# Danderson123/Amira

Measured on AMD Instinct MI355X. Metric: gene-mers/s to corrected GeneMerGraph, higher is better.
Workload: dtype int32; 1 GPU; synthetic 1M reads x 60 genes, k=5, 20k-gene vocab: build + error-correction sweep (build, filter(3,1), correct, build, clip(5), correct, build); reads_per_gpu=1000000, genes_per_read=60, k=5, vocab=20000, gene_mers_per_gpu=56000000, final_nodes=472478, final_edges=1054844, multi_gpu=n/a

## Files before the change

### amira_amd/csrc/amg_correct.h

```cpp
#pragma once
#include "amg_device.h"

enum { RC_SKIP = 0, RC_COPY = 1, RC_DROP = 2, RC_TRIM = 3, RC_GAPPED = 4, RC_KEEP_ORIG = 5 };

struct CorrArgs {
  const int* tokens;
  const long long* read_off;
  const int* tok_node;
  const signed char* tok_dir;
  const unsigned char* read_fix;
  const long long* p0s;
  const long long* p0e;
  const long long* p1s;
  const long long* p1e;
  long long n0;
  const long long* pos_off;
  const long long* read_len;
  long long n_reads;
  int k, flip, have_pos;
  unsigned int* gflag;
  unsigned long long* max_bound;
  unsigned long long* lmask;
  unsigned long long* n_runs;
  unsigned char* cls;
// ... 36 lines not shown

__device__ __forceinline__ unsigned long long gap_run_ends(unsigned long long lv, int start, int end) {
  const unsigned long long inside =
      (end >= 63 ? ~0ull : ((1ull << (end + 1)) - 1ull)) & ~((1ull << (start & 63)) - 1ull);
  return ~lv & inside & (lv >> 1);
}
__device__ __forceinline__ void gap_run_terminals(unsigned long long lv, int i, int& ps, int& pe) {
  ps = 63 - __clzll((long long)(lv & ((1ull << i) - 1ull)));
  pe = i + 1;
}

struct GapArgs {
  CorrArgs a;
  GView g;
  const GapRec* rec;
  const int* gapped_reads;
  long long n_gapped;
  int* pool;
  unsigned long long pool_cap;
  unsigned long long* pool_used;
  unsigned long long* status;
  int* cand;
  unsigned int cand_stride;
  unsigned char* final_cls;
  unsigned char* need_slow;
  const int* gq;
  const int4* qres;
  const int* qpool;
};

#define GF_MAXW 128
#define GF_MAXGAP 16
#define GF_POOL 384
#define GF_CAND 136
#define GF_MAXCOMBO 256
#define GM_INLINE 64
#define LEAN_CHUNK 32
#define CLS_READS 64
#define PACK_READS 64
enum {
  GS_NOT_TRIED = 1,
  GS_WINDOWS = 2,
  GS_RUNS = 3,
  GS_MEMO_UNFIT = 4,
  GS_RECORDS = 5,
  GS_COMBOS = 6,
  GS_CAND = 7,
  GS_CODES = 8
};
enum {
  GL_NO_SLOTS = 1,
  GL_ANSWERS = 2,
  GL_LONG = 3,
  GL_OTHER = 4,
  GL_CODES = 5
};

#define NWF_MAX_M 64
#define NWF_MAX_N 128
__device__ __forceinline__ bool nw_fast_ok(long long N, long long M) {
  return N <= NWF_MAX_N && M <= NWF_MAX_M && N > 0 && M > 0;
}

struct __attribute__((aligned(16))) NwRec {
  int r, M, N, pad;
  long long t0, dst;
  long long pdst;
  long long poff;
};

struct NwArgs {
  CorrArgs a;
  const NwRec* rec;
  long long* o_gs;
  long long* o_ge;
  const int* gapped_reads;
  long long n_gapped;
  const unsigned char* final_cls;
  const long long* big_off;
  unsigned char* big_buf;
  int allow_fast;
  int shortcuts;
  unsigned char* route;
};
enum { NW_ROUTE_NONE = 0, NW_ROUTE_EQUAL = 1, NW_ROUTE_CERT = 2, NW_ROUTE_FILL = 3, NW_ROUTE_LDS = 4, NW_ROUTE_GLOBAL = 5 };

struct PackArgs {
  CorrArgs a;
  const long long* new_idx;
  const long long* new_off;
  const unsigned char* final_cls;
  int* o_tok;
  long long* o_off;
  int* o_orig;
  unsigned char* o_changed;
  long long* o_src;
  const long long* pos_new;
  long long* o_posoff;
  long long* o_rl;
  long long out_reads, out_tokens;
  unsigned long long* dead_kept;
};

struct CorrSwitches {
  bool gap_memo;
  bool fast_gapped;
  bool lean_gapped;
  int fast_nw;
  int nw_shortcuts;
  const char* node_bound;
  bool routes;
  const char* gap_pool;
  const char* memo_spill;
};

struct CorrScratch {
  size_t per_read = 0;
  unsigned char *cls = nullptr, *final_cls = nullptr;
  int *r_start = nullptr, *r_end = nullptr;
  long long *nw_size = nullptr, *nw_off = nullptr;
  unsigned int *bound = nullptr, *new_len = nullptr, *flag = nullptr;
  long long *tmp_off = nullptr, *new_idx = nullptr, *new_off = nullptr;
  int* tmp_tok = nullptr;
  long long *plen = nullptr, *poffs = nullptr, *pos_new = nullptr;
  unsigned long long *max_bound = nullptr, *n_general = nullptr;
  unsigned long long* n_runs = nullptr;
  unsigned long long* dead_kept = nullptr;
  bool count_alive = false;
  DevBuf* glist = nullptr;
  DevBuf* cand = nullptr;
  DevBuf* pool = nullptr;
  DevBuf* need_slow = nullptr;
};

struct CorrCounts {
  long long tmp_total = 0, n_gapped = 0, total_runs = 0;
  unsigned long long max_bound = 0;
  bool carry = false;
  long long out_reads = 0, out_tokens = 0, big_total = 0, pos_total = 0;
  unsigned long long n_general = 0;
  long long n_queries = 0;
  int pool_retries = 0;
  bool lean_ran = false, fast_ran = false, memo = false;
};

static void fill_pos_args(amg_ctx* c, CorrArgs& a) {
  a.p0s = c->have_pos ? c->gene_start.as<long long>() : nullptr;
  a.p0e = c->have_pos ? c->gene_end.as<long long>() : nullptr;
  a.p1s = c->pos1_s.as<long long>();
  a.p1e = c->pos1_e.as<long long>();
  a.n0 = c->pos_n0;
  a.pos_off = (c->have_pos && !c->pos_identity) ? c->pos_off.as<long long>() : nullptr;
}

void corr_classify_launch(amg_ctx* c, const CorrArgs& a);
int corr_gapped(amg_ctx* c, const CorrSwitches& sw, const CorrScratch& S, const CorrArgs& a, CorrCounts& n);
int corr_nw_sizes(amg_ctx* c, const CorrSwitches& sw, const CorrScratch& S, const CorrArgs& a, long long n_gapped,
                  FetchList& shape);
int corr_grow_pos_pools(amg_ctx* c, const CorrCounts& n);
int corr_positions(amg_ctx* c, const CorrSwitches& sw, const CorrScratch& S, const CorrArgs& a, const CorrCounts& n,
                   unsigned char* route = nullptr);

int routes_begin(amg_ctx* c);
int routes_gapped(amg_ctx* c, const CorrScratch& S, const CorrCounts& n, const unsigned char* need_slow, const int* gq);
int routes_nw(amg_ctx* c, const CorrScratch& S, const CorrCounts& n);
int routes_end(amg_ctx* c, const CorrCounts& n);
```

### amira_amd/csrc/amg_correct.hip

```cpp
#include "amg_correct.h"

__global__ __launch_bounds__(256) void k_count_alive(const unsigned char* __restrict__ alive, long long n,
                                                     unsigned long long* out) {
  __shared__ unsigned int s_part[4];
  unsigned int c = 0;
  for (long long i = ((long long)blockIdx.x * blockDim.x + threadIdx.x) * 4; i < n; i += (long long)gridDim.x * blockDim.x * 4) {
    if (i + 4 <= n) {
      const unsigned int w = *reinterpret_cast<const unsigned int*>(alive + i);
      c += __popc(w & 0x01010101u);
    } else {
      for (long long j = i; j < n; ++j) c += alive[j] ? 1u : 0u;
    }
  }
  for (int d = 32; d > 0; d >>= 1) c += (unsigned int)__shfl_xor((int)c, d, 64);
  if ((threadIdx.x & 63) == 0) s_part[threadIdx.x >> 6] = c;
  __syncthreads();
  if (threadIdx.x == 0 && (s_part[0] | s_part[1] | s_part[2] | s_part[3]))
    atomicAdd(out, (unsigned long long)s_part[0] + s_part[1] + s_part[2] + s_part[3]);
}

__global__ __launch_bounds__(256) void k_corr_pack(PackArgs A) {
  const CorrArgs& a = A.a;
  const int lane = threadIdx.x & 63;
  const long long r = ((long long)blockIdx.x * 4 + (threadIdx.x >> 6)) * PACK_READS + lane;
  if (blockIdx.x == 0 && threadIdx.x == 0) A.o_off[A.out_reads] = A.out_tokens;
  long long dst = 0, src = 0;
  int n = 0;
  unsigned int dead = 0;
  if (r < a.n_reads && a.new_len[r] > 0) {
    dst = A.new_off[r];
    n = (int)a.new_len[r];
    const unsigned char fc = A.final_cls[r];
    if (fc == RC_KEEP_ORIG) {
      const long long nw = a.read_off[r + 1] - a.read_off[r] - a.k + 1;
      dead = nw <= 64 ? (unsigned int)(nw - __popcll(a.lmask[r])) : (unsigned int)nw;
    }
    long long poff = 0;
    if (fc == RC_GAPPED) {
      src = a.tmp_off[r] | (1ll << 62);
      if (a.have_pos) poff = A.pos_new[r];
    } else {
      const long long cut = fc == RC_TRIM ? a.r_start[r] : 0;
      src = a.read_off[r] + cut;
      if (a.have_pos) poff = (a.pos_off ? a.pos_off[r] : a.read_off[r]) + cut;
    }
    const long long q = A.new_idx[r];
    A.o_off[q] = dst;
    A.o_orig[q] = (int)r;
    A.o_changed[q] = (fc == RC_TRIM || fc == RC_GAPPED) ? 1 : 0;
    A.o_src[q] = fc == RC_GAPPED ? -1ll : src;
    if (a.have_pos) A.o_posoff[q] = poff;
    if (a.read_len) A.o_rl[q] = a.read_len[r];
  }
  if (__ballot(dead != 0u) != 0ull) {
    for (int d = 32; d > 0; d >>= 1) dead += (unsigned int)__shfl_xor((int)dead, d, 64);
    if (lane == 0) atomicAdd(A.dead_kept + 16 * (blockIdx.x & 15), (unsigned long long)dead);
  }
  if (__ballot(n > 0) == 0ull) return;
  for (int j0 = 0; j0 < PACK_READS; j0 += 4) {
    const int* sp[4];
    long long d[4];
    int nn[4], vt[4];
#pragma unroll
    for (int j = 0; j < 4; ++j) {
      nn[j] = __builtin_amdgcn_readlane(n, j0 + j);
      const long long sj = bcast_i64(src, j0 + j);
      d[j] = bcast_i64(dst, j0 + j);
      sp[j] = ((sj >> 62) & 1 ? a.tmp_tok : a.tokens) + (sj & ~(1ll << 62));
    }
#pragma unroll
    for (int j = 0; j < 4; ++j)
      if (lane < nn[j]) vt[j] = sp[j][lane];
#pragma unroll
    for (int j = 0; j < 4; ++j)
      if (lane < nn[j]) A.o_tok[d[j] + lane] = vt[j];
#pragma unroll
    for (int j = 0; j < 4; ++j)
      for (int i = 64 + lane; i < nn[j]; i += 64)
        A.o_tok[d[j] + i] = sp[j][i];
  }
}

static CorrSwitches read_switches() {
  auto is_one = [](const char* name) {
    const char* v = getenv(name);
    return v && v[0] == '1';
  };
  CorrSwitches sw;
  sw.gap_memo = !is_one("AMG_NO_GAP_MEMO");
  sw.fast_gapped = !is_one("AMG_NO_FAST_GAPPED");
  sw.lean_gapped = !is_one("AMG_NO_LEAN_GAPPED");
  sw.fast_nw = !is_one("AMG_NO_FAST_NW");
  sw.nw_shortcuts = !is_one("AMG_NW_NO_SHORTCUT");
  sw.node_bound = getenv("AMG_TEST_NODE_BOUND");
  sw.routes = is_one("AMG_CORR_ROUTES");
  sw.gap_pool = getenv("AMG_TEST_GAP_POOL");
  sw.memo_spill = getenv("AMG_TEST_MEMO_SPILL");
  return sw;
}

static int plan_per_read(amg_ctx* c, CorrScratch& S) {
  const size_t per_read = (size_t)(c->n_reads + 2);
  AMGCHK(c->s0.ensure(per_read * (1 + 1) + 64));
  AMGCHK(c->s1.ensure(per_read * sizeof(int) * 2 + per_read * sizeof(long long) * 2 + 64));
  AMGCHK(c->s2.ensure(per_read * sizeof(unsigned int) * 3));
  AMGCHK(c->s3.ensure(per_read * sizeof(long long) * 3));
  AMGCHK(c->gm_mask.ensure(per_read * sizeof(unsigned long long)));
  AMGCHK(c->gm_ctr.ensure((16 + 256 + 256 + 16) * sizeof(unsigned long long)));
  S.per_read = per_read;
  S.cls = c->s0.as<unsigned char>();
  S.final_cls = S.cls + per_read;
  S.r_start = c->s1.as<int>();
  S.r_end = S.r_start + per_read;
  S.nw_size = reinterpret_cast<long long*>(((uintptr_t)(S.r_end + per_read) + 15) & ~(uintptr_t)15);
  S.nw_off = S.nw_size + per_read;
  S.bound = c->s2.as<unsigned int>();
  S.new_len = S.bound + per_read;
  S.flag = S.new_len + per_read;
  S.tmp_off = c->s3.as<long long>();
  S.new_idx = S.tmp_off + per_read;
  S.new_off = S.new_idx + per_read;
  S.max_bound = S.n_general = c->status.as<unsigned long long>() + ST_MISC;
  S.n_runs = c->gm_ctr.as<unsigned long long>() + 16;
  S.dead_kept = S.n_runs + 256;
  S.count_alive = c->n_nodes >= (1ll << 20);
  S.glist = &c->c_orig;
  S.cand = &c->c_gstart;
  S.pool = &c->c_gend;
  S.need_slow = &c->c_changed;
  return AMG_OK;
}

static int plan_staging(amg_ctx* c, CorrScratch& S, long long tmp_total) {
  AMGCHK(c->c_tokens_buf.ensure((size_t)(tmp_total + 4) * sizeof(int)));
  AMGCHK(c->s4.ensure((size_t)(tmp_total + 4) * sizeof(int)));
  S.tmp_tok = c->s4.as<int>();
  return AMG_OK;
}

static int plan_positions(amg_ctx* c, CorrScratch& S, long long n_gapped) {
  AMGCHK(c->s5.ensure((size_t)(2 * (n_gapped + 2) + c->n_reads + 2) * sizeof(long long)));
  S.plen = c->s5.as<long long>();
  S.poffs = S.plen + (n_gapped + 2);
  S.pos_new = S.poffs + (n_gapped + 2);
  return AMG_OK;
}

static void corr_args(amg_ctx* c, const CorrScratch& S, CorrArgs& a) {
  a.tokens = c->tokens.as<int>();
  a.read_off = c->read_off.as<long long>();
  a.tok_node = c->tok_node.as<int>();
  a.tok_dir = c->tok_dir.as<signed char>();
  a.read_fix = c->read_fix.as<unsigned char>();
  fill_pos_args(c, a);
  a.read_len = c->have_read_len ? c->read_len.as<long long>() : nullptr;
  a.n_reads = c->n_reads;
  a.k = c->k;
  a.flip = c->two_v - 1;
  a.have_pos = c->have_pos ? 1 : 0;
  a.gflag = S.flag;
  a.max_bound = S.max_bound;
  a.lmask = c->gm_mask.as<unsigned long long>();
  a.n_runs = S.n_runs;
  a.cls = S.cls;
  a.cls_final = S.final_cls;
  a.r_start = S.r_start;
  a.r_end = S.r_end;
  a.bound = S.bound;
  a.tmp_off = S.tmp_off;
  a.new_len = S.new_len;
  a.tmp_tok = S.tmp_tok;
}

static int corr_classify(amg_ctx* c, const CorrScratch& S, const CorrArgs& a, CorrCounts& n) {
  hipStream_t st = c->stream;
  const long long R = c->n_reads;
// ... 156 lines not shown
```

### amira_amd/csrc/amg_correct_nw.hip

```cpp
#include "amg_correct.h"

#define NW_LDS_N 1024
#define NW_LDS_CELLS 16384
__global__ __launch_bounds__(64) void k_corr_nw(NwArgs A) {
  __shared__ unsigned char s_ptr[NW_LDS_CELLS];
  __shared__ int s_diag[3 * (NW_LDS_N + 1)];
  __shared__ unsigned char s_ops[2 * NW_LDS_N];
  const CorrArgs& a = A.a;
  const long long gi = blockIdx.x;
  if (gi >= A.n_gapped) return;
  const long long r = A.rec[gi].r;
  const long long pdst = A.rec[gi].pdst;
  if (A.final_cls[r] == RC_KEEP_ORIG) return;
  const int lane = threadIdx.x;
  const long long t0 = a.read_off[r];
  const int M = (int)(a.read_off[r + 1] - t0);
  const int N = (int)a.new_len[r];
  if (A.allow_fast && nw_fast_ok(N, M)) return;
  const long long dst = a.tmp_off[r];
  const int* x = a.tmp_tok + dst;
  const int* y = a.tokens + t0;
  const long long *ogs, *oge;
  pos_base(a, A.rec[gi].poff, ogs, oge);
  unsigned char* P = s_ptr;
  int* dg = s_diag;
  unsigned char* ops = s_ops;
  const bool small = (N <= NW_LDS_N && M <= NW_LDS_N && (long long)N * M <= NW_LDS_CELLS);
  if (!small) {
    unsigned char* base = A.big_buf + A.big_off[gi];
    P = base;
    ops = base + (long long)N * M;
    dg = reinterpret_cast<int*>(base + (((long long)N * M + N + M + 15) & ~15ll));
  }
  int* d0 = dg;
  int* d1 = d0 + (N + 1);
  int* d2 = d1 + (N + 1);
  for (int d = 0; d <= N + M - 2; ++d) {
    int ilo = d - (M - 1) > 0 ? d - (M - 1) : 0;
    int ihi = d < N - 1 ? d : N - 1;
    for (int i = ilo + lane; i <= ihi; i += 64) {
      int j = d - i;
      int f_dd = (i == 0 && j == 0) ? 0 : (i == 0 ? -(j - 1) : (j == 0 ? -(i - 1) : d0[i]));
      int f_im1 = (i == 0) ? -j : d1[i];
      int f_jm1 = (j == 0) ? -i : d1[i + 1];
      int s_diag_ = f_dd + (x[i] == y[j] ? 1 : 0);
      int s_left = f_im1 - 1;
      int s_up = f_jm1 - 1;
      int best = s_diag_;
      unsigned char ptr = 0;
      if (s_left >= best) { best = s_left; ptr = 1; }
      if (s_up >= best) { best = s_up; ptr = 2; }
      d2[i + 1] = best;
      P[(long long)i * M + j] = ptr;
    }
    __syncthreads();
    int* t = d0; d0 = d1; d1 = d2; d2 = t;
  }
  if (lane != 0) return;
  int n_ops = 0;
  int i = N - 1, j = M - 1;
  while (i >= 0 && j >= 0) {
    unsigned char p = P[(long long)i * M + j];
    ops[n_ops++] = p;
    if (p == 0) { --i; --j; }
    else if (p == 1) --i;
    else --j;
  }
  while (i >= 0) { ops[n_ops++] = 1; --i; }
  while (j >= 0) { ops[n_ops++] = 2; --j; }
  const long long NONE = (long long)0x8000000000000000ull;
  int xi = 0, yj = 0, cur = 0, out = 0;
  for (int o = n_ops - 1; o >= 0; --o) {
    unsigned char p = ops[o];
    if (p == 0) {
      if (x[xi] == y[yj]) {
        A.o_gs[pdst + out] = ogs[cur];
        A.o_ge[pdst + out] = oge[cur];
        ++cur;
      } else {
        A.o_gs[pdst + out] = NONE;
        A.o_ge[pdst + out] = NONE;
      }
      ++out; ++xi; ++yj;
    } else if (p == 1) {
      A.o_gs[pdst + out] = NONE;
      A.o_ge[pdst + out] = NONE;
      ++out; ++xi;
    } else {
      ++cur; ++yj;
    }
  }
  long long prev_end = 0;
  const long long rl = a.read_len ? a.read_len[r] : 0;
  for (int q = 0; q < N; ++q) {
    long long sv = A.o_gs[pdst + q], ev = A.o_ge[pdst + q];
    if (ev != NONE) prev_end = ev;
    if (sv == NONE && ev == NONE) {
      long long nxt = NONE;
      for (int w = q + 1; w < N; ++w)
        if (A.o_gs[pdst + w] != NONE) { nxt = A.o_gs[pdst + w]; break; }
      A.o_gs[pdst + q] = prev_end;
      A.o_ge[pdst + q] = (nxt != NONE) ? nxt : rl - 1;
    }
  }
}



#define NWF_WPB 1
struct NwfLds {
  int x[NWF_MAX_N];
  unsigned int opw[(NWF_MAX_N + NWF_MAX_M) / 16 + 1];
  long long gs[NWF_MAX_N];
  long long ge[NWF_MAX_N];
  long long ogs[NWF_MAX_M];
  long long oge[NWF_MAX_M];
};

__device__ __forceinline__ void nw_fast_read(const NwArgs& A, long long gi, int lane, NwfLds& S) {
  int (*s_x)[NWF_MAX_N] = &S.x;
  unsigned int (*s_opw)[(NWF_MAX_N + NWF_MAX_M) / 16 + 1] = &S.opw;
  long long (*s_gs)[NWF_MAX_N] = &S.gs;
  long long (*s_ge)[NWF_MAX_N] = &S.ge;
  long long (*s_ogs)[NWF_MAX_M] = &S.ogs;
  long long (*s_oge)[NWF_MAX_M] = &S.oge;
  const CorrArgs& a = A.a;
  const int wv = 0;
  const NwRec q = A.rec[gi];
  const int N = __builtin_amdgcn_readfirstlane(q.N);
  if (N == 0) return;
  const int M = __builtin_amdgcn_readfirstlane(q.M);
  const long long r = q.r, t0 = q.t0, dst = q.dst, pdst = q.pdst;
  int* X = s_x[wv];
  unsigned int* OPW = s_opw[wv];
  long long* GS = s_gs[wv];
  long long* GE = s_ge[wv];
  long long* OGS = s_ogs[wv];
  long long* OGE = s_oge[wv];
  const int x0 = lane < N ? a.tmp_tok[dst + lane] : -2;
  const int x1 = lane + 64 < N ? a.tmp_tok[dst + lane + 64] : -2;
  const int yj = lane < M ? a.tokens[t0 + lane] : -1;
  const long long *pgs, *pge;
  pos_base(a, q.poff, pgs, pge);
  const long long ogs = lane < M ? pgs[lane] : 0;
  const long long oge = lane < M ? pge[lane] : 0;
  const long long rl = a.read_len ? a.read_len[r] : 0;
  if (lane < N) X[lane] = x0;
  if (lane + 64 < N) X[lane + 64] = x1;
  OGS[lane] = ogs;
  OGE[lane] = oge;
  const long long NONE = (long long)0x8000000000000000ull;
  bool diagonal = false;
  int route = NW_ROUTE_FILL;
  if (N == M) {
    const unsigned long long mm = __ballot(lane < N && x0 != yj);
    const int m = __popcll(mm);
    diagonal = m <= 1;
    const int x_next = __shfl_down(x0, 1, 64), y_next = __shfl_down(yj, 1, 64);
    const unsigned long long eq_a = __ballot(lane < N - 1 && x0 == y_next);
    const unsigned long long eq_b = __ballot(lane < N - 1 && x_next == yj);
    if (m == 2) {
      const int b = 63 - __clzll((long long)mm);
      const unsigned long long upto_b = (1ull << b) - 1ull;
      diagonal = (eq_a & upto_b) != upto_b && (eq_b & upto_b) != upto_b;
    } else if (m == 3 || m == 4) {
      const unsigned long long dmask = ~mm & (N == 64 ? ~0ull : ((1ull << N) - 1ull));
      const unsigned long long below = (1ull << lane) - 1ull;
      const int prefD = __popcll(dmask & below);
      const int sufD = lane >= 63 ? 0 : __popcll(dmask >> (lane + 1));
      const int ID = (int)0x80000000 / 2;
      int best = ID;
#pragma unroll
      for (int side = 0; side < 2; ++side) {
        const int prefS = __popcll((side == 0 ? eq_a : eq_b) & below);
        int g = lane < N ? prefD - prefS + (lane == 0 ? 1 : 0) : ID;
        g = max(g, __builtin_amdgcn_update_dpp(ID, g, 0x111, 0xf, 0xf, false));
        g = max(g, __builtin_amdgcn_update_dpp(ID, g, 0x112, 0xf, 0xf, false));
        g = max(g, __builtin_amdgcn_update_dpp(ID, g, 0x114, 0xf, 0xf, false));
        g = max(g, __builtin_amdgcn_update_dpp(ID, g, 0x118, 0xf, 0xf, false));
        g = max(g, __builtin_amdgcn_update_dpp(ID, g, 0x142, 0xa, 0xf, false));
        g = max(g, __builtin_amdgcn_update_dpp(ID, g, 0x143, 0xc, 0xf, false));
        int h = lane < N ? g + prefS + sufD - 2 : ID;
        for (int d = 32; d > 0; d >>= 1) h = max(h, __shfl_xor(h, d, 64));
        best = max(best, h);
      }
      diagonal = best < N - m;
    }
    diagonal = diagonal && A.shortcuts != 0;
    if (diagonal) route = NW_ROUTE_EQUAL;
    if (diagonal && lane < N) {
      const bool match = ((mm >> lane) & 1ull) == 0ull;
      const int cur = __popcll(~mm & ((1ull << lane) - 1ull));
      GS[lane] = match ? OGS[cur] : NONE;
      GE[lane] = match ? OGE[cur] : NONE;
    }
  }
  if (!diagonal && A.shortcuts != 0 && N <= M && N >= 2) {
    int s_off = 0x7fffffff;
    bool ok = true;
    unsigned long long matched = 0ull;
    for (int i = 0; i < N && ok; ++i) {
      const int g = __builtin_amdgcn_readlane(x0, i);
      const unsigned long long at = __ballot(lane < M && yj == g);
      if (at != 0ull) {
        const int si = __ffsll((long long)at) - 1 - i;
        ok = (at & (at - 1ull)) == 0ull && (s_off == 0x7fffffff || si == s_off);
        s_off = si;
        matched |= 1ull << i;
      }
    }
    ok = ok && s_off != 0x7fffffff && s_off >= 0 && s_off <= M - N && __popcll(matched) >= 2;
    if (ok) {
      diagonal = true;
      route = NW_ROUTE_CERT;
      if (lane < N) {
// ... 37 lines not shown
    {
      int i = N - 1, j = M - 1;
      unsigned int pack = 0;
  #pragma unroll
      for (int blk = NWF_MAX_N / 16 - 1; blk >= 0; --blk) {
        while (i >= blk * 16 && j >= 0) {
          const unsigned int w = (unsigned int)__builtin_amdgcn_readlane((int)ptrs[blk], j);
          const unsigned int p = (w >> ((i & 15) * 2)) & 3u;
          pack |= p << ((n_ops & 15) * 2);
          if ((n_ops & 15) == 15) {
            if (lane == 0) OPW[n_ops >> 4] = pack;
            pack = 0;
          }
          ++n_ops;
          if (p == 0) { --i; --j; }
          else if (p == 1) --i;
          else --j;
        }
      }
      while (i >= 0) {
        pack |= 1u << ((n_ops & 15) * 2);
        if ((n_ops & 15) == 15) {
          if (lane == 0) OPW[n_ops >> 4] = pack;
          pack = 0;
        }
        ++n_ops;
        --i;
      }
      while (j >= 0) {
        pack |= 2u << ((n_ops & 15) * 2);
        if ((n_ops & 15) == 15) {
          if (lane == 0) OPW[n_ops >> 4] = pack;
          pack = 0;
        }
        ++n_ops;
        --j;
      }
      if ((n_ops & 15) != 0 && lane == 0) OPW[n_ops >> 4] = pack;
    }
    wave_sync();
    int base_x = 0, base_y = 0, base_cur = 0;
    for (int c0 = 0; c0 < n_ops; c0 += 64) {
      const int f = c0 + lane;
      const bool in = f < n_ops;
      const int g = in ? n_ops - 1 - f : 0;
      const unsigned int op = in ? (OPW[g >> 4] >> ((g & 15) * 2)) & 3u : 3u;
      const bool isx = in && (op == 0 || op == 1), isy = in && (op == 0 || op == 2);
      const unsigned long long lt = (1ull << lane) - 1ull;
      const unsigned long long bx = __ballot(isx), by = __ballot(isy);
      const int xi = base_x + __popcll(bx & lt), yy = base_y + __popcll(by & lt);
      const int ysel = __shfl(yj, yy < 64 ? yy : 0, 64);
      const bool match = in && op == 0 && X[xi < NWF_MAX_N ? xi : 0] == ysel;
      const bool inc = in && (op == 2 || match);
      const unsigned long long bc = __ballot(inc);
      const int cur = base_cur + __popcll(bc & lt);
      if (isx) {
        GS[xi] = match ? OGS[cur < NWF_MAX_M ? cur : 0] : NONE;
        GE[xi] = match ? OGE[cur < NWF_MAX_M ? cur : 0] : NONE;
      }
      base_x += __popcll(bx);
      base_y += __popcll(by);
      base_cur += __popcll(bc);
    }
  }
  wave_sync();
  if (A.route && lane == 0) A.route[gi] = (unsigned char)route;
  for (int q = lane; q < N; q += 64) {
    long long sv = GS[q], ev = GE[q];
    if (sv == NONE && ev == NONE) {
      long long prev_end = 0;
      for (int w = q - 1; w >= 0; --w)
        if (GE[w] != NONE) { prev_end = GE[w]; break; }
      long long nxt = NONE;
      for (int w = q + 1; w < N; ++w)
        if (GS[w] != NONE) { nxt = GS[w]; break; }
      sv = prev_end;
      ev = (nxt != NONE) ? nxt : rl - 1;
    }
    A.o_gs[pdst + q] = sv;
    A.o_ge[pdst + q] = ev;
  }
}

__global__ __launch_bounds__(64 * NWF_WPB) void k_corr_nw_fast(NwArgs A) {
  __shared__ NwfLds s_lds;
  if ((long long)blockIdx.x < A.n_gapped) nw_fast_read(A, (long long)blockIdx.x, (int)threadIdx.x, s_lds);
}

__global__ void k_nw_sizes(const int* __restrict__ gapped, long long n_gapped,
                           const long long* __restrict__ read_off, const unsigned int* __restrict__ new_len,
                           const long long* __restrict__ tmp_off, const long long* __restrict__ new_off,
                           const unsigned char* __restrict__ final_cls, long long* __restrict__ size,
                           int allow_fast, unsigned long long* n_general, NwRec* __restrict__ rec,
                           const long long* __restrict__ pos_off, long long* __restrict__ plen) {
  long long gi = (long long)blockIdx.x * blockDim.x + threadIdx.x;
  if (gi >= n_gapped) return;
  long long r = gapped[gi];
  long long N = new_len[r], M = read_off[r + 1] - read_off[r];
  {
    NwRec q;
    q.r = (int)r;
    q.M = (int)(M > 0x7fffffff ? 0x7fffffff : M);
    q.N = (final_cls[r] != RC_KEEP_ORIG && allow_fast && nw_fast_ok(N, M)) ? (int)N : 0;
    q.pad = 0;
    q.t0 = read_off[r];
    q.dst = tmp_off[r];
    q.pdst = 0;
    q.poff = pos_off ? pos_off[r] : read_off[r];
    rec[gi] = q;
    plen[gi] = final_cls[r] != RC_KEEP_ORIG ? N : 0;
  }
  bool small = (N <= NW_LDS_N && M <= NW_LDS_N && N * M <= NW_LDS_CELLS);
  long long bytes = 0;
  if (!small && final_cls[r] != RC_KEEP_ORIG)
    bytes = ((N * M + N + M + 15) & ~15ll) + ((3 * (N + 1) * 4 + 15) & ~15ll);
  size[gi] = bytes;
  if (final_cls[r] != RC_KEEP_ORIG && !(allow_fast && nw_fast_ok(N, M))) atomicAdd(n_general, 1ull);
}


__global__ void k_nw_place(long long n_gapped, const long long* __restrict__ poffs, long long base, long long n0,
                           NwRec* __restrict__ rec, long long* __restrict__ pos_new) {
  long long gi = (long long)blockIdx.x * blockDim.x + threadIdx.x;
  if (gi >= n_gapped) return;
  const long long at = base + poffs[gi];
  rec[gi].pdst = at;
  pos_new[rec[gi].r] = n0 + at;
}

static int grow_keep(amg_ctx* c, DevBuf& b, size_t need, size_t used) {
  if (need <= b.cap && !b.borrowed) return AMG_OK;
  DevBuf nb;
  AMGCHK(nb.ensure(need + need / 2));
  if (used && b.p) HIPCHK(hipMemcpyAsync(nb.p, b.p, used, hipMemcpyDeviceToDevice, c->stream));
  HIPCHK(hipStreamSynchronize(c->stream));
  b.release();
  b = nb;
  return AMG_OK;
}

int corr_nw_sizes(amg_ctx* c, const CorrSwitches& sw, const CorrScratch& S, const CorrArgs& a, long long n_gapped,
                  FetchList& shape) {
  {
    ClearList cl;
    cl.add(S.nw_size, (size_t)(n_gapped + 1) * sizeof(long long));
    cl.add(S.plen, (size_t)(n_gapped + 1) * sizeof(long long));
    cl.add(S.n_general, sizeof(unsigned long long));
    AMGCHK(clear_many(c, cl));
  }
  AMGCHK(c->nw_rec.ensure((size_t)(n_gapped + 1) * sizeof(NwRec)));
  hipLaunchKernelGGL(k_nw_sizes, dim3(nblk(n_gapped, 256)), dim3(256), 0, c->stream, S.glist->as<int>(),
                     n_gapped, a.read_off, S.new_len, S.tmp_off, S.new_off, S.final_cls, S.nw_size, sw.fast_nw,
                     S.n_general, c->nw_rec.as<NwRec>(), a.pos_off, S.plen);
  AMGCHK(prim_exscan_i64_pair(c, S.nw_size, S.nw_off, S.plen, S.poffs, (size_t)n_gapped));
  shape.add(S.nw_off + n_gapped);
  shape.add(S.poffs + n_gapped);
  shape.add(S.n_general);
  return AMG_OK;
}

int corr_grow_pos_pools(amg_ctx* c, const CorrCounts& n) {
  AMGCHK(c->nw_big.ensure((size_t)n.big_total + 64));
  const size_t used = (size_t)c->pos1_used * sizeof(long long);
  const size_t need = (size_t)(c->pos1_used + n.pos_total + 64) * sizeof(long long);
  AMGCHK(grow_keep(c, c->pos1_s, need, used));
  AMGCHK(grow_keep(c, c->pos1_e, need, used));
  return AMG_OK;
}

int corr_positions(amg_ctx* c, const CorrSwitches& sw, const CorrScratch& S, const CorrArgs& a, const CorrCounts& n,
                   unsigned char* route) {
  hipStream_t st = c->stream;
  const long long n_gapped = n.n_gapped;
  hipLaunchKernelGGL(k_nw_place, dim3(nblk(n_gapped, 256)), dim3(256), 0, st, n_gapped, S.poffs,
                     (long long)c->pos1_used, (long long)c->pos_n0, c->nw_rec.as<NwRec>(), S.pos_new);
  NwArgs W;
  W.a = a;
  W.rec = c->nw_rec.as<NwRec>();
  W.o_gs = c->pos1_s.as<long long>();
  W.o_ge = c->pos1_e.as<long long>();
  W.gapped_reads = nullptr;
  W.n_gapped = n_gapped;
  W.final_cls = S.final_cls;
  W.big_off = S.nw_off;
  W.big_buf = c->nw_big.as<unsigned char>();
  W.allow_fast = sw.fast_nw;
  W.shortcuts = sw.nw_shortcuts;
  W.route = route;
  if (W.allow_fast)
    hipLaunchKernelGGL(k_corr_nw_fast, dim3((unsigned int)n_gapped), dim3(64 * NWF_WPB), 0, st, W);
  if (n.n_general > 0)
    hipLaunchKernelGGL(k_corr_nw, dim3((unsigned int)n_gapped), dim3(64), 0, st, W);
  return AMG_OK;
}

struct NwProbeLoan {
  amg_ctx* c;
  DevBuf gene_start, gene_end, pos_off, pos1_s, pos1_e;
  bool have_pos, pos_identity;
  int64_t pos_n0, pos1_used;
  explicit NwProbeLoan(amg_ctx* ctx)
      : c(ctx), gene_start(ctx->gene_start), gene_end(ctx->gene_end), pos_off(ctx->pos_off), pos1_s(ctx->pos1_s),
        pos1_e(ctx->pos1_e), have_pos(ctx->have_pos), pos_identity(ctx->pos_identity), pos_n0(ctx->pos_n0),
        pos1_used(ctx->pos1_used) {
    c->gene_start = c->gene_end = c->pos_off = c->pos1_s = c->pos1_e = DevBuf();
  }
  ~NwProbeLoan() {
    c->gene_start.release(), c->gene_end.release(), c->pos_off.release(), c->pos1_s.release(), c->pos1_e.release();
    c->gene_start = gene_start, c->gene_end = gene_end, c->pos_off = pos_off, c->pos1_s = pos1_s, c->pos1_e = pos1_e;
    c->have_pos = have_pos, c->pos_identity = pos_identity, c->pos_n0 = pos_n0, c->pos1_used = pos1_used;
  }
};
struct NwProbeBufs {
  DevBuf tokens, read_off, tmp_tok, tmp_off, new_len, final_cls, read_len, glist, sizes, places, route;
  ~NwProbeBufs() {
    for (DevBuf* b : {&tokens, &read_off, &tmp_tok, &tmp_off, &new_len, &final_cls, &read_len, &glist, &sizes, &places,
                      &route})
      b->release();
  }
};
static int probe_up(DevBuf& b, const void* src, size_t bytes, size_t room = 0) {
  AMGCHK(b.ensure(bytes + room + 16));
  if (bytes) HIPCHK(hipMemcpy(b.p, src, bytes, hipMemcpyHostToDevice));
  return AMG_OK;
}

#define NWP_GUARD 64
#define NWP_GUARD_PRE 8
#define NWP_N0_POOLED 5
extern "C" int amg_nw_probe(amg_ctx* c, int64_t n_pairs, const int32_t* x_tok, const int64_t* x_off, const int32_t* y_tok,
                            const int64_t* y_off, const int64_t* y_start, const int64_t* y_end, const int64_t* read_len,
                            const uint8_t* keep_orig, int flags, int64_t* out_start, int64_t* out_end, uint8_t* route,
                            int64_t* state) {
  if (!c || n_pairs < 1 || n_pairs > (1ll << 20) || !x_off || !y_tok || !y_off || !y_start || !y_end || !route || !state ||
      flags < 0 || flags > 7 || x_off[0] != 0 || y_off[0] != 0)
    return amg_fail(AMG_E_ARG, "nw_probe: bad arguments");
  long long want_pos = 0, want_big = 0;
  for (int64_t p = 0; p < n_pairs; ++p) {
    const long long N = x_off[p + 1] - x_off[p], M = y_off[p + 1] - y_off[p];
    const bool keep = keep_orig && keep_orig[p];
    if (N < 0 || M < 1 || (N < 1 && !keep) || N > (1 << 24) || M > (1 << 24))
      return amg_fail(AMG_E_ARG, "nw_probe: pair %lld has %lld corrected and %lld original genes", (long long)p, N, M);
    if (keep) continue;
    want_pos += N;
    if (!(N <= NW_LDS_N && M <= NW_LDS_N && N * M <= NW_LDS_CELLS)) want_big += N * M + 16 * (N + M) + 64;
    if (want_big > (1ll << 30)) return amg_fail(AMG_E_ARG, "nw_probe: more than 1 GiB of matrix scratch");
  }
  const long long total_x = x_off[n_pairs], total_y = y_off[n_pairs];
  if (total_x > 0 && !x_tok) return amg_fail(AMG_E_ARG, "nw_probe: no corrected genes");
  if (want_pos > 0 && (!out_start || !out_end)) return amg_fail(AMG_E_ARG, "nw_probe: no room for the positions");
  for (long long i = 0; i < total_x; ++i)
    if (x_tok[i] < 0) return amg_fail(AMG_E_ARG, "nw_probe: negative corrected gene at %lld", i);
  for (long long i = 0; i < total_y; ++i)
    if (y_tok[i] < 0) return amg_fail(AMG_E_ARG, "nw_probe: negative original gene at %lld", i);
  HIPCHK(hipSetDevice(c->device));

  const bool pooled = (flags & 4) != 0;
  NwProbeLoan loan(c);
  NwProbeBufs B;
  CorrSwitches sw = {};
  sw.fast_nw = (flags & 1) ? 0 : 1;
  sw.nw_shortcuts = (flags & 2) ? 0 : 1;
  std::vector<unsigned int> new_len((size_t)n_pairs);
  std::vector<unsigned char> cls((size_t)n_pairs);
  std::vector<int> glist((size_t)n_pairs);
  for (int64_t p = 0; p < n_pairs; ++p) {
    new_len[p] = (unsigned int)(x_off[p + 1] - x_off[p]);
    cls[p] = (keep_orig && keep_orig[p]) ? RC_KEEP_ORIG : RC_GAPPED;
    glist[p] = (int)p;
  }
  const size_t np1 = (size_t)n_pairs + 1;
  AMGCHK(probe_up(B.tokens, y_tok, (size_t)total_y * 4));
  AMGCHK(probe_up(B.read_off, y_off, np1 * 8));
  AMGCHK(probe_up(B.tmp_tok, x_tok, (size_t)total_x * 4, NWP_GUARD * 4));
  HIPCHK(hipMemset(B.tmp_tok.as<int>() + total_x, 0xff, NWP_GUARD * 4));
  AMGCHK(probe_up(B.tmp_off, x_off, np1 * 8));
  AMGCHK(probe_up(B.new_len, new_len.data(), (size_t)n_pairs * 4));
  AMGCHK(probe_up(B.final_cls, cls.data(), (size_t)n_pairs));
  if (read_len) AMGCHK(probe_up(B.read_len, read_len, (size_t)n_pairs * 8));
  AMGCHK(probe_up(B.glist, glist.data(), (size_t)n_pairs * 4));
  AMGCHK(B.sizes.ensure((n_pairs + 2) * 2 * sizeof(long long)));
  AMGCHK(B.places.ensure((n_pairs + 2) * 3 * sizeof(long long)));
  AMGCHK(B.route.ensure((size_t)n_pairs + 16));
  HIPCHK(hipMemset(B.route.p, 0, (size_t)n_pairs));
  const long long used = (pooled ? total_y : 0) + NWP_GUARD_PRE;
  {
    std::vector<long long> ps((size_t)used, -1ll), pe((size_t)used, -1ll);
    if (pooled) {
      memcpy(ps.data(), y_start, (size_t)total_y * 8);
      memcpy(pe.data(), y_end, (size_t)total_y * 8);
      const long long filler[NWP_N0_POOLED] = {-1, -1, -1, -1, -1};
      std::vector<long long> off((size_t)n_pairs);
      for (int64_t p = 0; p < n_pairs; ++p) off[p] = NWP_N0_POOLED + y_off[p];
      AMGCHK(probe_up(c->gene_start, filler, sizeof(filler)));
      AMGCHK(probe_up(c->gene_end, filler, sizeof(filler)));
      AMGCHK(probe_up(c->pos_off, off.data(), (size_t)n_pairs * 8));
    } else {
      AMGCHK(probe_up(c->gene_start, y_start, (size_t)total_y * 8));
      AMGCHK(probe_up(c->gene_end, y_end, (size_t)total_y * 8));
    }
    AMGCHK(c->pos1_s.ensure((size_t)used * 8));
    AMGCHK(c->pos1_e.ensure((size_t)used * 8));
    HIPCHK(hipMemcpy(c->pos1_s.p, ps.data(), (size_t)used * 8, hipMemcpyHostToDevice));
    HIPCHK(hipMemcpy(c->pos1_e.p, pe.data(), (size_t)used * 8, hipMemcpyHostToDevice));
  }
  c->have_pos = true;
  c->pos_identity = !pooled;
  c->pos_n0 = pooled ? NWP_N0_POOLED : total_y;
  c->pos1_used = used;
  HIPCHK(hipDeviceSynchronize());

  CorrScratch S;
  S.per_read = (size_t)n_pairs + 2;
  S.final_cls = B.final_cls.as<unsigned char>();
  S.nw_size = B.sizes.as<long long>();
  S.nw_off = S.nw_size + (n_pairs + 2);
  S.new_len = B.new_len.as<unsigned int>();
  S.tmp_off = B.tmp_off.as<long long>();
  S.tmp_tok = B.tmp_tok.as<int>();
  S.plen = B.places.as<long long>();
  S.poffs = S.plen + (n_pairs + 2);
  S.pos_new = S.poffs + (n_pairs + 2);
  S.n_general = c->status.as<unsigned long long>() + ST_MISC;
  S.glist = &B.glist;
  CorrArgs a;
  memset(&a, 0, sizeof(a));
  a.tokens = B.tokens.as<int>();
  a.read_off = B.read_off.as<long long>();
  fill_pos_args(c, a);
  a.read_len = read_len ? B.read_len.as<long long>() : nullptr;
  a.n_reads = n_pairs;
  a.have_pos = 1;
  a.cls_final = S.final_cls;
  a.tmp_off = S.tmp_off;
  a.new_len = S.new_len;
  a.tmp_tok = S.tmp_tok;
  CorrCounts n;
  n.n_gapped = n_pairs;
  n.carry = true;
  FetchList shape;
  AMGCHK(corr_nw_sizes(c, sw, S, a, n_pairs, shape));
  unsigned long long v[3] = {0, 0, 0};
  AMGCHK(fetch(c, shape, v));
// ... 46 lines not shown
```

Baseline: 10.28 billion gene-mers/s.

## Stream easy NW alignments through persistent prefetching waves before fast-path kernel

Adds a persistent streaming kernel with a fixed number of single-wave blocks. Each block walks gapped reads with a stride, prefetches record batches and token/position rows several items ahead, and settles diagonal or certified alignments directly, also folding in the position-placement kernel. Reads it cannot settle are marked in a todo array. The fast NW kernel then handles only those, packing several waves per block and assigning todo items by ballot. This is meant to replace one block per gapped read and hide load latency, at the cost of more code and an extra todo buffer.

Result: no change. 10.25 billion gene-mers/s (-0.3%).

```diff
diff --git a/amira_amd/csrc/amg_correct.h b/amira_amd/csrc/amg_correct.h
--- a/amira_amd/csrc/amg_correct.h
+++ b/amira_amd/csrc/amg_correct.h
@@ -142,7 +142,15 @@
   int allow_fast;
   int shortcuts;
   unsigned char* route;
-};
+  const long long* poffs;
+  long long pbase;
+  long long* pos_new;
+  unsigned char* todo;
+  long long waves;
+};
+__device__ __forceinline__ long long nw_pdst(const NwArgs& A, long long gi, const NwRec& q) {
+  return A.poffs ? A.pbase + A.poffs[gi] : q.pdst;
+}
 enum { NW_ROUTE_NONE = 0, NW_ROUTE_EQUAL = 1, NW_ROUTE_CERT = 2, NW_ROUTE_FILL = 3, NW_ROUTE_LDS = 4, NW_ROUTE_GLOBAL = 5 };
 
 struct PackArgs {
@@ -168,11 +176,15 @@
   bool lean_gapped;
   int fast_nw;
   int nw_shortcuts;
+  bool stream_nw;
+  const char* nw_waves;
   const char* node_bound;
   bool routes;
   const char* gap_pool;
   const char* memo_spill;
 };
+
+CorrSwitches read_switches();
 
 struct CorrScratch {
   size_t per_read = 0;
diff --git a/amira_amd/csrc/amg_correct.hip b/amira_amd/csrc/amg_correct.hip
--- a/amira_amd/csrc/amg_correct.hip
+++ b/amira_amd/csrc/amg_correct.hip
@@ -81,7 +81,7 @@
   }
 }
 
-static CorrSwitches read_switches() {
+CorrSwitches read_switches() {
   auto is_one = [](const char* name) {
     const char* v = getenv(name);
     return v && v[0] == '1';
@@ -92,6 +92,8 @@
   sw.lean_gapped = !is_one("AMG_NO_LEAN_GAPPED");
   sw.fast_nw = !is_one("AMG_NO_FAST_NW");
   sw.nw_shortcuts = !is_one("AMG_NW_NO_SHORTCUT");
+  sw.stream_nw = !is_one("AMG_NO_STREAM_NW");
+  sw.nw_waves = getenv("AMG_TEST_NW_WAVES");
   sw.node_bound = getenv("AMG_TEST_NODE_BOUND");
   sw.routes = is_one("AMG_CORR_ROUTES");
   sw.gap_pool = getenv("AMG_TEST_GAP_POOL");
diff --git a/amira_amd/csrc/amg_correct_nw.hip b/amira_amd/csrc/amg_correct_nw.hip
--- a/amira_amd/csrc/amg_correct_nw.hip
+++ b/amira_amd/csrc/amg_correct_nw.hip
@@ -10,7 +10,7 @@
   const long long gi = blockIdx.x;
   if (gi >= A.n_gapped) return;
   const long long r = A.rec[gi].r;
-  const long long pdst = A.rec[gi].pdst;
+  const long long pdst = nw_pdst(A, gi, A.rec[gi]);
   if (A.final_cls[r] == RC_KEEP_ORIG) return;
   const int lane = threadIdx.x;
   const long long t0 = a.read_off[r];
@@ -107,7 +107,6 @@
 
 
 
-#define NWF_WPB 1
 struct NwfLds {
   int x[NWF_MAX_N];
   unsigned int opw[(NWF_MAX_N + NWF_MAX_M) / 16 + 1];
@@ -130,7 +129,7 @@
   const int N = __builtin_amdgcn_readfirstlane(q.N);
   if (N == 0) return;
   const int M = __builtin_amdgcn_readfirstlane(q.M);
-  const long long r = q.r, t0 = q.t0, dst = q.dst, pdst = q.pdst;
+  const long long r = q.r, t0 = q.t0, dst = q.dst, pdst = nw_pdst(A, gi, q);
   int* X = s_x[wv];
   unsigned int* OPW = s_opw[wv];
   long long* GS = s_gs[wv];
@@ -334,9 +333,210 @@
   }
 }
 
-__global__ __launch_bounds__(64 * NWF_WPB) void k_corr_nw_fast(NwArgs A) {
-  __shared__ NwfLds s_lds;
-  if ((long long)blockIdx.x < A.n_gapped) nw_fast_read(A, (long long)blockIdx.x, (int)threadIdx.x, s_lds);
+#define NWF_WAVES 4
+#define NWF_CHUNK 256
+__global__ __launch_bounds__(64 * NWF_WAVES) void k_corr_nw_fast(NwArgs A) {
+  extern __shared__ __attribute__((aligned(16))) unsigned char s_raw[];
+  NwfLds* s_lds = reinterpret_cast<NwfLds*>(s_raw);
+  const int lane = (int)threadIdx.x & 63, wv = (int)threadIdx.x >> 6;
+  if (!A.todo) {
+    if ((long long)blockIdx.x < A.n_gapped) nw_fast_read(A, (long long)blockIdx.x, lane, s_lds[0]);
+    return;
+  }
+  int k = 0;
+  for (int part = 0; part < NWF_CHUNK; part += 64) {
+    const long long base = (long long)blockIdx.x * NWF_CHUNK + part;
+    unsigned long long todo = __ballot(base + lane < A.n_gapped && A.todo[base + lane] != 0);
+    while (todo) {
+      const int b = __ffsll((long long)todo) - 1;
+      todo &= todo - 1ull;
+      if (k++ % NWF_WAVES != wv) continue;
+      nw_fast_read(A, base + b, lane, s_lds[wv]);
+      wave_sync();
+    }
+  }
+}
+
+#define NWS_WAVES 4096
+#define NWS_AHEAD 3
+struct NwsRec { int r, M, N; long long t0, dst, poff, pd; };
+struct NwsRow { int x, y; long long gs, ge, rl; };
+
+__device__ __forceinline__ int nws_recs(const NwArgs& A, long long g0, int lane) {
+  long long g = g0 + (long long)(lane >> 4) * A.waves;
+  g = g < A.n_gapped ? g : A.n_gapped - 1;
+  const int d = lane & 15;
+  const int* p = d < 12 ? reinterpret_cast<const int*>(A.rec + g) + d
+                        : reinterpret_cast<const int*>(A.poffs + g) + (d < 14 ? d - 12 : 1);
+  return *p;
+}
+__device__ __forceinline__ long long nws_word2(int b, int at) {
+  const unsigned int lo = (unsigned int)__builtin_amdgcn_readlane(b, at), hi = (unsigned int)__builtin_amdgcn_readlane(b, at + 1);
+  return (long long)(((unsigned long long)hi << 32) | lo);
+}
+__device__ __forceinline__ NwsRec nws_rec(int b, int j, bool in_list) {
+  NwsRec q;
+  q.r = __builtin_amdgcn_readlane(b, 16 * j + 0);
+  q.M = __builtin_amdgcn_readlane(b, 16 * j + 1);
+  q.N = in_list ? __builtin_amdgcn_readlane(b, 16 * j + 2) : 0;
+  q.t0 = nws_word2(b, 16 * j + 4);
+  q.dst = nws_word2(b, 16 * j + 6);
+  q.poff = nws_word2(b, 16 * j + 10);
+  q.pd = nws_word2(b, 16 * j + 12);
+  return q;
+}
+__device__ __forceinline__ bool nws_mine(const NwsRec& q) { return q.N >= 1 && q.N <= q.M && q.M <= NWF_MAX_M; }
+
+__device__ __forceinline__ void nws_row(const NwArgs& A, const NwsRec& q, int lane, NwsRow& w) {
+  const CorrArgs& a = A.a;
+  const bool mine = nws_mine(q);
+  const unsigned int lx = mine ? min(lane, q.N - 1) : 0, ly = mine ? min(lane, q.M - 1) : 0;
+  const long long *pgs, *pge;
+  pos_base(a, mine ? q.poff : 0, pgs, pge);
+  w.x = (a.tmp_tok + (mine ? q.dst : 0))[lx];
+  w.y = (a.tokens + (mine ? q.t0 : 0))[ly];
+  w.gs = pgs[ly];
+  w.ge = pge[ly];
+  w.rl = *(a.read_len ? a.read_len + (mine ? q.r : 0) : a.read_off);
+}
+
+__device__ __forceinline__ void nws_settle(const NwArgs& A, long long gi, const NwsRec& q, const NwsRow& w, int lane) {
+  const int N = q.N, M = q.M;
+  const long long pdst = A.pbase + q.pd;
+  if (lane == 0) A.pos_new[q.r] = A.a.n0 + pdst;
+  if (N == 0) {
+    if (lane == 0) A.todo[gi] = 0;
+    return;
+  }
+  const long long NONE = (long long)0x8000000000000000ull;
+  const int x0 = lane < N ? w.x : -2, yj = lane < M ? w.y : -1;
+  bool diagonal = false;
+  int route = NW_ROUTE_FILL;
+  int cur = 0;
+  bool match = false;
+  const bool mine = nws_mine(q);
+  if (mine && N == M) {
+    const unsigned long long mm = __ballot(lane < N && x0 != yj);
+    const int m = __popcll(mm);
+    diagonal = m <= 1;
+    if (m >= 2 && m <= 4) {
+      const int x_next = __shfl_down(x0, 1, 64), y_next = __shfl_down(yj, 1, 64);
+      const unsigned long long eq_a = __ballot(lane < N - 1 && x0 == y_next);
+      const unsigned long long eq_b = __ballot(lane < N - 1 && x_next == yj);
+      if (m == 2) {
+        const int b = 63 - __clzll((long long)mm);
+        const unsigned long long upto_b = (1ull << b) - 1ull;
+        diagonal = (eq_a & upto_b) != upto_b && (eq_b & upto_b) != upto_b;
+      } else {
+        const unsigned long long dmask = ~mm & (N == 64 ? ~0ull : ((1ull << N) - 1ull));
+        const unsigned long long below = (1ull << lane) - 1ull;
+        const int prefD = __popcll(dmask & below);
+        const int sufD = lane >= 63 ? 0 : __popcll(dmask >> (lane + 1));
+        const int ID = (int)0x80000000 / 2;
+        int best = ID;
+#pragma unroll
+        for (int side = 0; side < 2; ++side) {
+          const int prefS = __popcll((side == 0 ? eq_a : eq_b) & below);
+          int g = lane < N ? prefD - prefS + (lane == 0 ? 1 : 0) : ID;
+          g = max(g, __builtin_amdgcn_update_dpp(ID, g, 0x111, 0xf, 0xf, false));
+          g = max(g, __builtin_amdgcn_update_dpp(ID, g, 0x112, 0xf, 0xf, false));
+          g = max(g, __builtin_amdgcn_update_dpp(ID, g, 0x114, 0xf, 0xf, false));
+          g = max(g, __builtin_amdgcn_update_dpp(ID, g, 0x118, 0xf, 0xf, false));
+          g = max(g, __builtin_amdgcn_update_dpp(ID, g, 0x142, 0xa, 0xf, false));
+          g = max(g, __builtin_amdgcn_update_dpp(ID, g, 0x143, 0xc, 0xf, false));
+          int h = lane < N ? g + prefS + sufD - 2 : ID;
+          for (int d = 32; d > 0; d >>= 1) h = max(h, __shfl_xor(h, d, 64));
+          best = max(best, h);
+        }
+        diagonal = best < N - m;
+      }
+    }
+    if (diagonal) {
+      route = NW_ROUTE_EQUAL;
+      match = lane < N && ((mm >> lane) & 1ull) == 0ull;
+      cur = __popcll(~mm & ((1ull << lane) - 1ull));
+    }
+  }
+  if (mine && !diagonal && N >= 2) {
+    int s_off = 0x7fffffff;
+    bool ok = true;
+    unsigned long long matched = 0ull;
+    int yr = yj, cnt = 0, at_r = 0;
+#pragma unroll 8
+    for (int r = 0; r < 64; ++r) {
+      const bool eq = x0 == yr;
+      cnt += eq ? 1 : 0;
+      at_r = eq ? r : at_r;
+      yr = __builtin_amdgcn_update_dpp(0, yr, 0x134, 0xf, 0xf, false);
+    }
+    matched = __ballot(cnt == 1);
+    const int si = lane + at_r < 64 ? at_r : at_r - 64;
+    if (matched != 0ull) s_off = __builtin_amdgcn_readlane(si, __ffsll((long long)matched) - 1);
+    ok = __ballot(cnt > 1 || (cnt == 1 && si != s_off)) == 0ull;
+    ok = ok && s_off != 0x7fffffff && s_off >= 0 && s_off <= M - N && __popcll(matched) >= 2;
+    if (ok) {
+      diagonal = true;
+      route = NW_ROUTE_CERT;
+      match = lane < N && ((matched >> lane) & 1ull) != 0ull;
+      cur = s_off + __popcll(matched & ((1ull << lane) - 1ull));
+    }
+  }
+  if (lane == 0) A.todo[gi] = diagonal ? 0 : 1;
+  if (!diagonal) return;
+  if (A.route && lane == 0) A.route[gi] = (unsigned char)route;
+  long long ogs = w.gs, oge = w.ge;
+  if (__ballot(match && cur != lane) != 0ull) {
+    ogs = __shfl(w.gs, cur & 63, 64);
+    oge = __shfl(w.ge, cur & 63, 64);
+  }
+  long long sv = match ? ogs : NONE, ev = match ? oge : NONE;
+  const bool need = lane < N && sv == NONE && ev == NONE;
+  if (__ballot(need) != 0ull) {
+    const unsigned long long has_e = __ballot(lane < N && ev != NONE), has_s = __ballot(lane < N && sv != NONE);
+    const unsigned long long before = has_e & ((1ull << lane) - 1ull);
+    const unsigned long long after = lane >= 63 ? 0ull : has_s & ~((2ull << lane) - 1ull);
+    const long long prev_end = __shfl(ev, before ? 63 - __clzll((long long)before) : lane, 64);
+    const long long nxt = __shfl(sv, after ? __ffsll((long long)after) - 1 : lane, 64);
+    if (need) {
+      sv = before ? prev_end : 0;
+      ev = after ? nxt : (A.a.read_len ? w.rl : 0) - 1;
+    }
+  }
+  if (lane < N) {
+    (A.o_gs + pdst)[(unsigned int)lane] = sv;
+    (A.o_ge + pdst)[(unsigned int)lane] = ev;
+  }
+}
+
+__global__ __launch_bounds__(64) void k_corr_nw_stream(NwArgs A) {
+  constexpr int D = NWS_AHEAD, R = D + 1;
+  static_assert(4 % R == 0 && D >= 1, "NWS_AHEAD + 1 must divide the record batch");
+  const int lane = (int)threadIdx.x;
+  const long long G = A.waves, n = A.n_gapped;
+  long long gi = (G & 7) == 0 ? (long long)(blockIdx.x & 7) * (G >> 3) + (blockIdx.x >> 3) : blockIdx.x;
+  if (gi >= n) return;
+  int b0 = nws_recs(A, gi, lane);
+  int b1 = nws_recs(A, gi + 4 * G, lane);
+  NwsRow w[R];
+  NwsRec q[R];
+#pragma unroll
+  for (int j = 0; j < D; ++j) {
+    q[j] = nws_rec(b0, j, gi + j * G < n);
+    nws_row(A, q[j], lane, w[j]);
+  }
+  for (;;) {
+    const int b2 = nws_recs(A, gi + 8 * G, lane);
+#pragma unroll
+    for (int j = 0; j < 4; ++j) {
+      q[(j + D) % R] = nws_rec(j + D < 4 ? b0 : b1, (j + D) & 3, gi + D * G < n);
+      nws_row(A, q[(j + D) % R], lane, w[(j + D) % R]);
+      nws_settle(A, gi, q[j % R], w[j % R], lane);
+      gi += G;
+      if (gi >= n) return;
+    }
+    b0 = b1;
+    b1 = b2;
+  }
 }
 
 __global__ void k_nw_sizes(const int* __restrict__ gapped, long long n_gapped,
@@ -400,7 +600,7 @@
     cl.add(S.n_general, sizeof(unsigned long long));
     AMGCHK(clear_many(c, cl));
   }
-  AMGCHK(c->nw_rec.ensure((size_t)(n_gapped + 1) * sizeof(NwRec)));
+  AMGCHK(c->nw_rec.ensure((size_t)(n_gapped + 1) * sizeof(NwRec) + (size_t)n_gapped + 64));
   hipLaunchKernelGGL(k_nw_sizes, dim3(nblk(n_gapped, 256)), dim3(256), 0, c->stream, S.glist->as<int>(),
                      n_gapped, a.read_off, S.new_len, S.tmp_off, S.new_off, S.final_cls, S.nw_size, sw.fast_nw,
                      S.n_general, c->nw_rec.as<NwRec>(), a.pos_off, S.plen);
@@ -424,8 +624,7 @@
                    unsigned char* route) {
   hipStream_t st = c->stream;
   const long long n_gapped = n.n_gapped;
-  hipLaunchKernelGGL(k_nw_place, dim3(nblk(n_gapped, 256)), dim3(256), 0, st, n_gapped, S.poffs,
-                     (long long)c->pos1_used, (long long)c->pos_n0, c->nw_rec.as<NwRec>(), S.pos_new);
+  const bool stream = sw.stream_nw && sw.fast_nw && sw.nw_shortcuts;
   NwArgs W;
   W.a = a;
   W.rec = c->nw_rec.as<NwRec>();
@@ -439,8 +638,23 @@
   W.allow_fast = sw.fast_nw;
   W.shortcuts = sw.nw_shortcuts;
   W.route = route;
-  if (W.allow_fast)
-    hipLaunchKernelGGL(k_corr_nw_fast, dim3((unsigned int)n_gapped), dim3(64 * NWF_WPB), 0, st, W);
+  W.poffs = stream ? S.poffs : nullptr;
+  W.pbase = (long long)c->pos1_used;
+  W.pos_new = S.pos_new;
+  W.todo = stream ? c->nw_rec.as<unsigned char>() + (size_t)(n_gapped + 1) * sizeof(NwRec) : nullptr;
+  W.waves = NWS_WAVES;
+  if (sw.nw_waves && atoll(sw.nw_waves) >= 1 && atoll(sw.nw_waves) < W.waves) W.waves = atoll(sw.nw_waves);
+  if (W.waves > n_gapped) W.waves = n_gapped;
+  if (stream) {
+    hipLaunchKernelGGL(k_corr_nw_stream, dim3((unsigned int)W.waves), dim3(64), 0, st, W);
+    hipLaunchKernelGGL(k_corr_nw_fast, dim3(nblk(n_gapped, NWF_CHUNK)), dim3(64 * NWF_WAVES), NWF_WAVES * sizeof(NwfLds),
+                       st, W);
+  } else {
+    hipLaunchKernelGGL(k_nw_place, dim3(nblk(n_gapped, 256)), dim3(256), 0, st, n_gapped, S.poffs,
+                       (long long)c->pos1_used, (long long)c->pos_n0, c->nw_rec.as<NwRec>(), S.pos_new);
+    if (W.allow_fast)
+      hipLaunchKernelGGL(k_corr_nw_fast, dim3((unsigned int)n_gapped), dim3(64), sizeof(NwfLds), st, W);
+  }
   if (n.n_general > 0)
     hipLaunchKernelGGL(k_corr_nw, dim3((unsigned int)n_gapped), dim3(64), 0, st, W);
   return AMG_OK;
@@ -510,7 +724,7 @@
   const bool pooled = (flags & 4) != 0;
   NwProbeLoan loan(c);
   NwProbeBufs B;
-  CorrSwitches sw = {};
+  CorrSwitches sw = read_switches();
   sw.fast_nw = (flags & 1) ? 0 : 1;
   sw.nw_shortcuts = (flags & 2) ? 0 : 1;
   std::vector<unsigned int> new_len((size_t)n_pairs);
```
